# QuantumLiquids/PEPS

Hardware: AMD Instinct MI355X
Metric: configuration-amplitudes/sec (higher is better)
Workload: dtype f32

## Files before the change

### include/pepsgpu.h

```cpp
#ifndef PEPSGPU_H
#define PEPSGPU_H

#include <stddef.h>
#include <stdint.h>

#ifdef __cplusplus
extern "C" {
#endif

typedef struct pepsgpu_ctx pepsgpu_ctx;

enum {
  PEPSGPU_OK = 0,
  PEPSGPU_EINVAL = 1,
  PEPSGPU_EHIP = 2,
  PEPSGPU_ESTATE = 3,
  PEPSGPU_ERANGE = 4,
  PEPSGPU_EEMPTY = 5
};
enum { PEPSGPU_F32 = 0, PEPSGPU_F64 = 1, PEPSGPU_C128 = 3 };
enum { PEPSGPU_LEFT = 0, PEPSGPU_DOWN = 1, PEPSGPU_RIGHT = 2, PEPSGPU_UP = 3 };
enum { PEPSGPU_HORIZONTAL = 0, PEPSGPU_VERTICAL = 1 };
enum { PEPSGPU_SVD_COMPRESS = 0, PEPSGPU_VARIATION2SITE = 1, PEPSGPU_VARIATION1SITE = 2 };

// ... 119 lines not shown
int pepsgpu_sr_weighted_sum(pepsgpu_ctx *ctx, const double *y, double *out);
int pepsgpu_sr_copy_samples(pepsgpu_ctx *ctx, void *dst_samples_dev, int32_t *dst_configs_dev);

int pepsgpu_update_local(pepsgpu_ctx *ctx, int n_sites, const int32_t *sites, const int32_t *new_states,
                         const uint8_t *accept_mask);
int pepsgpu_erase_envs_after_update(pepsgpu_ctx *ctx, int row, int col);

int pepsgpu_evaluate_amplitude(pepsgpu_ctx *ctx, double *out_amp);

int pepsgpu_walker_flags(pepsgpu_ctx *ctx, int32_t *flags_out);
int pepsgpu_sync(pepsgpu_ctx *ctx);
int pepsgpu_stats(pepsgpu_ctx *ctx, double *stats_out, int n);
int pepsgpu_profile_enable(pepsgpu_ctx *ctx, int on);
int pepsgpu_profile_read(pepsgpu_ctx *ctx, double *out);

int pepsgpu_comm_unique_id(void *id128_out);
int pepsgpu_comm_init(pepsgpu_ctx *ctx, int nranks, int rank, const void *id128);
int pepsgpu_comm_size(pepsgpu_ctx *ctx);
int pepsgpu_comm_rank(pepsgpu_ctx *ctx);
int pepsgpu_comm_destroy(pepsgpu_ctx *ctx);
int pepsgpu_allreduce(pepsgpu_ctx *ctx, void *buf, long n, int dtype, int op, int on_device);
int pepsgpu_grad_allreduce(pepsgpu_ctx *ctx);
int pepsgpu_bcast_state(pepsgpu_ctx *ctx, int root);
int pepsgpu_grad_device_ptr(pepsgpu_ctx *ctx, void **so_dev, void **seo_dev, long *n_elems);

int pepsgpu_diag_tgemm(int dtype_in, int dtype_out, const int *desc_ints, int n_ints, const void *A, size_t a_elems,
                       const void *B, size_t b_elems, void *C, size_t c_elems, int nbatch, long wA, long wB, long wC);
int pepsgpu_diag_tgemm_desc(int types, const int *desc_ints, int n_ints, const long *desc_longs, int n_longs,
                            const double *desc_dbls, int n_dbls, const int32_t *pool, long pool_n, const float *scale_in,
                            const void *A, size_t a_elems, long a_offset, const void *B, size_t b_elems, long b_offset,
                            void *C, size_t c_elems, float *scale_out, double *norm_log, int32_t *norm_flag,
                            int32_t *route_out, unsigned long long *flops_out);
int pepsgpu_diag_tgemm_route(int types, const int *desc_ints, int n_ints, const long *desc_longs, int n_longs,
                             const double *desc_dbls, int n_dbls, long a_offset, long b_offset, int32_t *route_out);
int pepsgpu_diag_tgemm_chain3(const int *dims8, const int *site_strides4, long slot, int nslots, const int32_t *sel, int sel_inc,
                              const int32_t *live4, const int32_t *skip, int nbatch, const int *offs3, const float *mps1,
                              const float *bten, const float *site, const float *mps2, float *out, int32_t *flags_out,
                              int32_t *launched_out, int32_t *variant_out);
int pepsgpu_diag_dot4(int dtype, const void *a, const void *b, const int *dims4, int nbatch, const double *lsum, const int32_t *flag,
                      double *out);
int pepsgpu_diag_chol(int dtype_out, const double *G, int n, int nbatch, void *R_out);
int pepsgpu_diag_gram_cols(int dtype, const void *P, int K, int n, int nbatch, const int32_t *klive, double *G_out);
int pepsgpu_diag_gram_rows(const float *M, int n, int K, int nbatch, const int32_t *nrows, double *G_out);
int pepsgpu_diag_mgemm_dense(const float *R, const float *Tt, int m, int la, int a_dim, int u_dim, int k2_dim, int tt_u_inner, int nbatch,
                             const int32_t *m_live, const int32_t *a_live, const int32_t *k2_live, float *M_out);
int pepsgpu_diag_cg_stats(double *out16);
int pepsgpu_diag_lds_gram_chol(int which, const float *X, int n, int K, int nbatch, const int32_t *nlive, float *R_out, int32_t *mlive_out);
int pepsgpu_diag_chol_pivot(const float *X, int n, int K, int nbatch, const int32_t *nlive, int kcap, float *R_out, int32_t *mlive_out);
int pepsgpu_diag_rows_qr(const float *X, int k, int len, int nbatch, const int32_t *klive, float *V_out, int32_t *klive_out);
int pepsgpu_diag_suwa_todo(const double *weights, int n, int init, const uint32_t *words, int steps, int32_t *out_chain);
int pepsgpu_diag_tgemm_chain(const int *dims7, const int32_t *live3_per_entry, int nbatch, const float *R, const float *A,
                             const float *W, float *P_out, int32_t *flags_out);
int pepsgpu_diag_gram_chol(int dtype, const void *P, int K, int n, int nbatch, void *R_out, int32_t *mlive_out);
int pepsgpu_diag_chol_adaptive(int dtype_out, const double *G, int n, int nbatch, void *R_out, int32_t *mlive_out);
int pepsgpu_diag_jacobi(int dtype, void *M, int m, int len, int nbatch, int k, void *Vt_out, void *S_out,
                        int force_global, int *sweeps_out);
const char *pepsgpu_version(void);

#ifdef __cplusplus
}
#endif
#endif
```

### peps_amd/capi.py

```python
import ctypes as C
import os

import numpy as np

_HERE = os.path.dirname(os.path.abspath(__file__))
LIB_PATH = os.environ.get("PEPSGPU_LIB") or os.path.join(_HERE, "lib", "libpepsgpu.so")

F32, F64 = 0, 1
C128 = 3
LEFT, DOWN, RIGHT, UP = 0, 1, 2, 3
HORIZONTAL, VERTICAL = 0, 1
LEFTUP_TO_RIGHTDOWN, LEFTDOWN_TO_RIGHTUP = 0, 1
SVD_COMPRESS, VARIATION2SITE, VARIATION1SITE = 0, 1, 2

_ERR = {1: ValueError, 2: RuntimeError, 3: RuntimeError, 4: IndexError, 5: RuntimeError}

SYMBOLS = [
    "pepsgpu_ctx_create", "pepsgpu_set_truncate_params", "pepsgpu_ctx_destroy", "pepsgpu_last_error", "pepsgpu_state_upload",
    "pepsgpu_walkers_set_configs", "pepsgpu_walkers_get_configs", "pepsgpu_n_walkers",
    "pepsgpu_grow_bmps_step", "pepsgpu_grow_full_bmps", "pepsgpu_grow_bmps_for_row", "pepsgpu_grow_bmps_for_col",
    "pepsgpu_shift_bmps_window", "pepsgpu_delete_inner_bmps", "pepsgpu_bmps_park", "pepsgpu_bmps_unpark", "pepsgpu_generate_bmps_approach",
    "pepsgpu_sweep_slice_exchange", "pepsgpu_sweep_slice_exchange_tab", "pepsgpu_sweep_slice_fullspace", "pepsgpu_sweep_slice_tnn3", "pepsgpu_diag_tnn3_table", "pepsgpu_nn_exchange_slice", "pepsgpu_nn_exchange_slice_tab", "pepsgpu_onsite_slice", "pepsgpu_nnn_exchange_slice", "pepsgpu_diag_nnn_slice_calls", "pepsgpu_nnn_hop_slice_fermion", "pepsgpu_diag_nnn_hop_slice_calls", "pepsgpu_diag_fermion_hop_cand", "pepsgpu_link_exchange_slice", "pepsgpu_diag_link_slice_calls", "pepsgpu_diag_link_cand", "pepsgpu_walker_create", "pepsgpu_walker_clone", "pepsgpu_walker_destroy", "pepsgpu_walker_info", "pepsgpu_walker_set_mpo", "pepsgpu_walker_set_mpo_excited", "pepsgpu_walker_trace_slice", "pepsgpu_diag_walker_slice_calls", "pepsgpu_walker_evolve",
    "pepsgpu_walker_evolve_step", "pepsgpu_walker_contract_row", "pepsgpu_walker_init_bten", "pepsgpu_walker_grow_bten_step",
    "pepsgpu_walker_shift_bten_window", "pepsgpu_walker_trace_with_bten", "pepsgpu_walker_clear_bten", "pepsgpu_walker_get_bmps_tensor",
    "pepsgpu_bmps_stack_size", "pepsgpu_get_bmps_tensor", "pepsgpu_init_bten", "pepsgpu_grow_full_bten",
    "pepsgpu_grow_bten_step", "pepsgpu_shift_bten_window", "pepsgpu_truncate_bten", "pepsgpu_bten_stack_size",
    "pepsgpu_trace", "pepsgpu_replace_nn_trace", "pepsgpu_replace_one_trace", "pepsgpu_punch_hole",
    "pepsgpu_init_bten2", "pepsgpu_grow_full_bten2", "pepsgpu_grow_bten2_step", "pepsgpu_shift_bten2_window",
    "pepsgpu_bten2_stack_size", "pepsgpu_replace_nnn_trace", "pepsgpu_replace_tnn_trace",
    "pepsgpu_bten2_select_set", "pepsgpu_cfg_override_slice", "pepsgpu_replace_plaquette_trace",
    "pepsgpu_replace_sqrt5_trace",
    "pepsgpu_grad_reset", "pepsgpu_grad_accumulate", "pepsgpu_grad_accumulate_states", "pepsgpu_grad_read", "pepsgpu_grad_device_ptr", "pepsgpu_grad_allreduce", "pepsgpu_bcast_state",
    "pepsgpu_comm_unique_id", "pepsgpu_comm_init", "pepsgpu_comm_size", "pepsgpu_comm_rank", "pepsgpu_comm_destroy",
    "pepsgpu_allreduce",
    "pepsgpu_sr_begin", "pepsgpu_sr_append", "pepsgpu_sr_count", "pepsgpu_sr_sum", "pepsgpu_sr_matvec", "pepsgpu_sr_matvec_c128",
    "pepsgpu_sr_cg_solve", "pepsgpu_sr_gram", "pepsgpu_sr_weighted_sum", "pepsgpu_sr_copy_samples",
    "pepsgpu_update_local", "pepsgpu_erase_envs_after_update", "pepsgpu_evaluate_amplitude",
    "pepsgpu_walker_flags", "pepsgpu_sync", "pepsgpu_stats", "pepsgpu_profile_enable", "pepsgpu_profile_read",
    "pepsgpu_diag_tgemm", "pepsgpu_diag_tgemm_desc", "pepsgpu_diag_tgemm_route", "pepsgpu_diag_tgemm_chain", "pepsgpu_diag_tgemm_chain3", "pepsgpu_diag_chol", "pepsgpu_diag_chol_adaptive", "pepsgpu_diag_chol_pivot", "pepsgpu_diag_rows_qr", "pepsgpu_diag_suwa_todo", "pepsgpu_diag_dot4", "pepsgpu_diag_gram_chol", "pepsgpu_diag_gram_cols", "pepsgpu_diag_gram_rows", "pepsgpu_diag_mgemm_dense", "pepsgpu_diag_jacobi", "pepsgpu_version",
]


def load_library(path=LIB_PATH):
    if not os.path.exists(path):
        raise ImportError("libpepsgpu.so not built (%s): run `python -c 'import __graft_entry__ as g; g.build()'`" % path)
    lib = C.CDLL(path)
    vp, ip, dp = C.c_void_p, C.POINTER(C.c_int32), C.POINTER(C.c_double)
    lib.pepsgpu_ctx_create.argtypes = [C.POINTER(vp)] + [C.c_int] * 8 + [C.c_double, C.c_int, C.c_int]
    lib.pepsgpu_set_truncate_params.argtypes = [vp, C.c_int, C.c_int, C.c_double, C.c_int, C.c_double, C.c_int]
    lib.pepsgpu_ctx_destroy.argtypes = [vp]
    lib.pepsgpu_ctx_destroy.restype = None
    lib.pepsgpu_last_error.argtypes = [vp]
    lib.pepsgpu_last_error.restype = C.c_char_p
    lib.pepsgpu_version.restype = C.c_char_p
    lib.pepsgpu_state_upload.argtypes = [vp, vp, C.c_int]
    lib.pepsgpu_walkers_set_configs.argtypes = [vp, C.c_int, ip]
    lib.pepsgpu_walkers_get_configs.argtypes = [vp, ip]
    lib.pepsgpu_n_walkers.argtypes = [vp]
    for name in ("grow_bmps_step", "grow_full_bmps", "grow_bmps_for_row", "grow_bmps_for_col", "shift_bmps_window",
                 "delete_inner_bmps", "generate_bmps_approach", "bmps_stack_size", "bten_stack_size",
                 "grow_bten_step", "shift_bten_window"):
        getattr(lib, "pepsgpu_" + name).argtypes = [vp, C.c_int]
    lib.pepsgpu_bmps_park.argtypes = [vp, C.c_int, C.c_int]
    lib.pepsgpu_bmps_unpark.argtypes = [vp, C.c_int]
    lib.pepsgpu_get_bmps_tensor.argtypes = [vp, C.c_int, C.c_int, C.c_int, ip, dp, dp]
    lib.pepsgpu_init_bten.argtypes = [vp, C.c_int, C.c_int]
    lib.pepsgpu_truncate_bten.argtypes = [vp, C.c_int, C.c_int]
    lib.pepsgpu_grow_full_bten.argtypes = [vp, C.c_int, C.c_int, C.c_int, C.c_int]
    lib.pepsgpu_trace.argtypes = [vp, C.c_int, C.c_int, C.c_int, dp]
    lib.pepsgpu_replace_nn_trace.argtypes = [vp, C.c_int, C.c_int, C.c_int, C.c_int, ip, dp]
    lib.pepsgpu_replace_one_trace.argtypes = [vp, C.c_int, C.c_int, C.c_int, C.c_int, ip, dp]
    lib.pepsgpu_punch_hole.argtypes = [vp, C.c_int, C.c_int, C.c_int, dp]
    for name in ("init_bten2", "grow_bten2_step", "shift_bten2_window"):
        getattr(lib, "pepsgpu_" + name).argtypes = [vp, C.c_int, C.c_int]
    lib.pepsgpu_grow_full_bten2.argtypes = [vp, C.c_int, C.c_int, C.c_int, C.c_int]
    lib.pepsgpu_bten2_stack_size.argtypes = [vp, C.c_int]
    lib.pepsgpu_replace_nnn_trace.argtypes = [vp, C.c_int, C.c_int, C.c_int, C.c_int, C.c_int, ip, dp]
    lib.pepsgpu_bten2_select_set.argtypes = [vp, C.c_int]
    lib.pepsgpu_cfg_override_slice.argtypes = [vp, C.c_int, C.c_int, ip]
    lib.pepsgpu_replace_plaquette_trace.argtypes = [vp, C.c_int, C.c_int, C.c_int, ip, C.c_int, C.c_int, dp]
    lib.pepsgpu_replace_tnn_trace.argtypes = [vp, C.c_int, C.c_int, C.c_int, C.c_int, ip, dp]
    lib.pepsgpu_replace_sqrt5_trace.argtypes = [vp, C.c_int, C.c_int, C.c_int, C.c_int, C.c_int, ip, dp]
    lib.pepsgpu_grad_reset.argtypes = [vp]
    lib.pepsgpu_grad_accumulate.argtypes = [vp, dp, dp, C.c_int]
    lib.pepsgpu_grad_accumulate_states.argtypes = [vp, dp, dp, C.c_int, ip]
    lib.pepsgpu_grad_read.argtypes = [vp, dp, dp]
    lib.pepsgpu_grad_device_ptr.argtypes = [vp, C.POINTER(vp), C.POINTER(vp), C.POINTER(C.c_long)]
    lib.pepsgpu_grad_allreduce.argtypes = [vp]
    lib.pepsgpu_bcast_state.argtypes = [vp, C.c_int]
    lib.pepsgpu_comm_unique_id.argtypes = [vp]
    lib.pepsgpu_comm_init.argtypes = [vp, C.c_int, C.c_int, vp]
    lib.pepsgpu_comm_size.argtypes = [vp]
# ... 658 lines not shown

def diag_tgemm_chain(R, A, W, live):
    R = np.ascontiguousarray(R, dtype=np.float32); A = np.ascontiguousarray(A, dtype=np.float32)
    W = np.ascontiguousarray(W, dtype=np.float32)
    nb, m, l, a = R.shape
    _, _, p, a2 = A.shape
    l2, u = W.shape[3], W.shape[4]
    dims = np.array([m, l, a, p, a2, l2, u], dtype=np.int32)
    lv = np.ascontiguousarray(live, dtype=np.int32)
    P = np.zeros((nb, m, u, l2, a2), dtype=np.float32)
    fl = np.zeros(nb, dtype=np.int32)
    f = lib().pepsgpu_diag_tgemm_chain
    f.argtypes = [C.POINTER(C.c_int32), C.POINTER(C.c_int32), C.c_int, C.c_void_p, C.c_void_p, C.c_void_p, C.c_void_p, C.POINTER(C.c_int32)]
    rc = f(_ip(dims), _ip(lv), nb, R.ctypes.data_as(C.c_void_p), A.ctypes.data_as(C.c_void_p), W.ctypes.data_as(C.c_void_p),
           P.ctypes.data_as(C.c_void_p), _ip(fl))
    if rc != 0:
        raise RuntimeError("diag_tgemm_chain failed: %s" % lib().pepsgpu_last_error(None).decode())
    return P, fl


def diag_chol(dtype_out, G):
    G = np.ascontiguousarray(G, dtype=np.float64)
    nb, n, _ = G.shape
    R = np.zeros((nb, n, n), dtype=np.float32 if dtype_out == F32 else np.float64)
    rc = lib().pepsgpu_diag_chol(dtype_out, _dp(G), n, nb, R.ctypes.data_as(C.c_void_p))
    if rc != 0:
        raise RuntimeError("diag_chol failed: %s" % lib().pepsgpu_last_error(None).decode())
    return R


def diag_chol_adaptive(dtype_out, G):
    G = np.ascontiguousarray(G, dtype=np.float64)
    nb, n, _ = G.shape
    R = np.zeros((nb, n, n), dtype=np.float32 if dtype_out == F32 else np.float64)
    ml = np.zeros(nb, dtype=np.int32)
    rc = lib().pepsgpu_diag_chol_adaptive(dtype_out, _dp(G), n, nb, R.ctypes.data_as(C.c_void_p), _ip(ml))
    if rc != 0:
        raise RuntimeError("diag_chol_adaptive failed: %s" % lib().pepsgpu_last_error(None).decode())
    return R, ml


def diag_gram_chol(dtype, P):
    t = np.float32 if dtype == F32 else np.float64
    P = np.ascontiguousarray(P, dtype=t)
    nb, K, n = P.shape
    R = np.zeros((nb, n, n), dtype=t)
    ml = np.zeros(nb, dtype=np.int32)
    rc = lib().pepsgpu_diag_gram_chol(dtype, P.ctypes.data_as(C.c_void_p), K, n, nb, R.ctypes.data_as(C.c_void_p), _ip(ml))
    if rc != 0:
        raise RuntimeError("diag_gram_chol failed: %s" % lib().pepsgpu_last_error(None).decode())
    return R, ml


def diag_gram_cols(dtype, P, klive=None):
    t = np.float32 if dtype == F32 else np.float64
    P = np.ascontiguousarray(P, dtype=t)
    nb, K, n = P.shape
    G = np.zeros((nb, n, n), dtype=np.float64)
    kl = None if klive is None else np.ascontiguousarray(klive, dtype=np.int32)
    f = lib().pepsgpu_diag_gram_cols
    f.argtypes = [C.c_int, C.c_void_p, C.c_int, C.c_int, C.c_int, C.POINTER(C.c_int32), C.POINTER(C.c_double)]
    rc = f(dtype, P.ctypes.data_as(C.c_void_p), K, n, nb, None if kl is None else _ip(kl), _dp(G))
    if rc != 0:
        raise RuntimeError("diag_gram_cols failed: %s" % lib().pepsgpu_last_error(None).decode())
    return G


def diag_gram_rows(M, nrows):
    M = np.ascontiguousarray(M, dtype=np.float32)
    nb, n, K = M.shape
    G = np.zeros((nb, n, n), dtype=np.float64)
    nr = np.ascontiguousarray(nrows, dtype=np.int32)
    f = lib().pepsgpu_diag_gram_rows
    f.argtypes = [C.c_void_p, C.c_int, C.c_int, C.c_int, C.POINTER(C.c_int32), C.POINTER(C.c_double)]
    rc = f(M.ctypes.data_as(C.c_void_p), n, K, nb, _ip(nr), _dp(G))
    if rc != 0:
        raise RuntimeError("diag_gram_rows failed: %s" % lib().pepsgpu_last_error(None).decode())
    return G


def diag_lds_gram_chol(which, X, nlive):
    X = np.ascontiguousarray(X, dtype=np.float32)
    nb = X.shape[0]
    n, K = (X.shape[1], X.shape[2]) if which == 0 else (X.shape[2], X.shape[1])
    R = np.zeros((nb, n, n), dtype=np.float32)
    ml = np.zeros(nb, dtype=np.int32)
    nl = np.ascontiguousarray(nlive, dtype=np.int32)
    f = lib().pepsgpu_diag_lds_gram_chol
    f.argtypes = [C.c_int, C.c_void_p, C.c_int, C.c_int, C.c_int, C.POINTER(C.c_int32), C.c_void_p, C.POINTER(C.c_int32)]
    rc = f(which, X.ctypes.data_as(C.c_void_p), n, K, nb, _ip(nl), R.ctypes.data_as(C.c_void_p), _ip(ml))
    if rc != 0:
        raise RuntimeError("diag_lds_gram_chol failed: %s" % lib().pepsgpu_last_error(None).decode())
    return R, ml


def diag_chol_pivot(X, nlive, kcap=64):
    X = np.ascontiguousarray(X, dtype=np.float32)
    nb, n, K = X.shape
    R = np.zeros((nb, kcap, n), dtype=np.float32)
    ml = np.zeros(nb, dtype=np.int32)
    nl = np.ascontiguousarray(nlive, dtype=np.int32)
    f = lib().pepsgpu_diag_chol_pivot
    f.argtypes = [C.c_void_p, C.c_int, C.c_int, C.c_int, C.POINTER(C.c_int32), C.c_int, C.c_void_p, C.POINTER(C.c_int32)]
    rc = f(X.ctypes.data_as(C.c_void_p), n, K, nb, _ip(nl), kcap, R.ctypes.data_as(C.c_void_p), _ip(ml))
    if rc != 0:
        raise RuntimeError("diag_chol_pivot failed: %s" % lib().pepsgpu_last_error(None).decode())
# ... 249 lines not shown
```

### peps_amd/csrc/capi.hip

```cpp
#include <cstring>
#include "../../include/pepsgpu.h"
#include "engine_impl.h"
#include "engine_nnn.h"
#include "engine_sr.h"
#include "engine_var.h"
#include "engine_cplx.h"
#include "engine_walker.h"
#include "engine_sweep.h"
#include "comm.h"

using namespace pepsgpu;

namespace pepsgpu {
bool tgemm_use_mfma() {
  static int v = -1;
  if (v < 0) {
    const char *e = getenv("PEPSGPU_NO_MFMA");
    v = (e && e[0] == '1') ? 0 : 1;
  }
  return v == 1;
}
}

struct pepsgpu_ctx {
// ... 681 lines not shown
  const size_t lsm = chol_lowrank_smem_bytes(n), smem = chol_smem_bytes(n);
  allow_dynamic_lds(reinterpret_cast<const void *>(&chol_lowrank_kernel<T>), lsm);
  allow_dynamic_lds(reinterpret_cast<const void *>(&chol_upper_kernel<T>), smem);
  hipLaunchKernelGGL(chol_lowrank_kernel<T>, dim3(nbatch), dim3(256), lsm, 0, (const double *)dG, (long)n * n, n, dR,
                     (long)n * n, dml);
  PG_CHECK_HIP(hipGetLastError());
  launch_chol_upper<T>(0, nbatch, dG, (long)n * n, n, dR, (long)n * n, dml, 1);
  PG_CHECK_HIP(hipGetLastError());
  PG_CHECK_HIP(hipDeviceSynchronize());
  PG_CHECK_HIP(hipMemcpy(Rout, dR, ne * sizeof(T), hipMemcpyDeviceToHost));
  PG_CHECK_HIP(hipMemcpy(mlive, dml, nbatch * sizeof(int), hipMemcpyDeviceToHost));
  (void)hipFree(dG); (void)hipFree(dR); (void)hipFree(dml);
}
extern "C" int pepsgpu_diag_chol_adaptive(int dtype_out, const double *G, int n, int nbatch, void *R_out, int32_t *mlive_out) {
  return guarded(nullptr, [&]() {
    if (dtype_out == 0) diag_chol_adaptive_t<float>(G, n, nbatch, R_out, mlive_out);
    else diag_chol_adaptive_t<double>(G, n, nbatch, R_out, mlive_out);
  });
}
template <typename T, int KCAP>
static void diag_gram_chol_t(const void *P, int K, int n, int nbatch, void *Rout, int32_t *mlive) {
  T *dP, *dR;
  int *dml;
  PG_REQUIRE(n <= 256, 1, "n too large for the fused low-rank kernel");
  PG_CHECK_HIP(hipMalloc(&dP, (size_t)K * n * nbatch * sizeof(T)));
  PG_CHECK_HIP(hipMalloc(&dR, (size_t)n * n * nbatch * sizeof(T)));
  PG_CHECK_HIP(hipMalloc(&dml, nbatch * sizeof(int)));
  PG_CHECK_HIP(hipMemcpy(dP, P, (size_t)K * n * nbatch * sizeof(T), hipMemcpyHostToDevice));
  PG_CHECK_HIP(hipMemset(dR, 0, (size_t)n * n * nbatch * sizeof(T)));
  const int npass = K > KCAP ? 4 : 1;
  std::vector<int> hk(nbatch, 0);
  for (int b = 0; b < nbatch; ++b)
    for (int r = 0; r < K; ++r) {
      const T *row = (const T *)P + ((size_t)b * K + r) * n;
      for (int c = 0; c < n; ++c)
        if (row[c] != T(0)) { hk[b] = r + 1; break; }
    }
  int *dk;
  PG_CHECK_HIP(hipMalloc(&dk, nbatch * sizeof(int)));
  PG_CHECK_HIP(hipMemcpy(dk, hk.data(), nbatch * sizeof(int), hipMemcpyHostToDevice));
  launch_gram_chol_lowrank<T, KCAP>(0, nbatch, (const T *)dP, (long)K * n, n, (const int *)dk, 1, K, dR, (long)n * n, dml, 1,
                                    (const int *)nullptr, npass);
  PG_CHECK_HIP(hipDeviceSynchronize());
  (void)hipFree(dk);
  PG_CHECK_HIP(hipDeviceSynchronize());
  PG_CHECK_HIP(hipMemcpy(Rout, dR, (size_t)n * n * nbatch * sizeof(T), hipMemcpyDeviceToHost));
  PG_CHECK_HIP(hipMemcpy(mlive, dml, nbatch * sizeof(int), hipMemcpyDeviceToHost));
  (void)hipFree(dP); (void)hipFree(dR); (void)hipFree(dml);
}
extern "C" int pepsgpu_diag_gram_chol(int dtype, const void *P, int K, int n, int nbatch, void *R_out, int32_t *mlive_out) {
  return guarded(nullptr, [&]() {
    if (dtype == 0) diag_gram_chol_t<float, 96>(P, K, n, nbatch, R_out, mlive_out);
    else diag_gram_chol_t<double, 48>(P, K, n, nbatch, R_out, mlive_out);
  });
}
template <typename T>
static void diag_gram_cols_t(const void *P, int K, int n, int nbatch, const int32_t *klive, double *G) {
  T *dP;
  double *dG;
  int *dk = nullptr;
  PG_CHECK_HIP(hipMalloc(&dP, (size_t)K * n * nbatch * sizeof(T)));
  PG_CHECK_HIP(hipMalloc(&dG, (size_t)n * n * nbatch * sizeof(double)));
  PG_CHECK_HIP(hipMemcpy(dP, P, (size_t)K * n * nbatch * sizeof(T), hipMemcpyHostToDevice));
  PG_CHECK_HIP(hipMemset(dG, 0, (size_t)n * n * nbatch * sizeof(double)));
  if (klive) {
    PG_CHECK_HIP(hipMalloc(&dk, nbatch * sizeof(int)));
    PG_CHECK_HIP(hipMemcpy(dk, klive, nbatch * sizeof(int), hipMemcpyHostToDevice));
  }
  launch_gram_cols_f64<T>(0, nbatch, (const T *)dP, (long)K * n, n, n, (const int *)dk, 1, K, dG, (const int *)nullptr, 1,
                          (const int *)nullptr, (unsigned long long *)nullptr, (unsigned long long *)nullptr);
  PG_CHECK_HIP(hipDeviceSynchronize());
  PG_CHECK_HIP(hipMemcpy(G, dG, (size_t)n * n * nbatch * sizeof(double), hipMemcpyDeviceToHost));
  (void)hipFree(dP); (void)hipFree(dG); if (dk) (void)hipFree(dk);
}
extern "C" int pepsgpu_diag_gram_cols(int dtype, const void *P, int K, int n, int nbatch, const int32_t *klive, double *G_out) {
  return guarded(nullptr, [&]() {
    PG_REQUIRE(K >= 1 && n >= 1 && n <= 256 && nbatch >= 1, 1, "bad sizes");
    if (dtype == 0) diag_gram_cols_t<float>(P, K, n, nbatch, klive, G_out); else diag_gram_cols_t<double>(P, K, n, nbatch, klive, G_out);
  });
}
extern "C" int pepsgpu_diag_gram_rows(const float *M, int n, int K, int nbatch, const int32_t *nrows, double *G_out) {
  return guarded(nullptr, [&]() {
    PG_REQUIRE(n >= 1 && n <= 256 && K >= 16 && K % 16 == 0 && nbatch >= 1 && nrows, 1, "bad sizes");
    float *dM; double *dG; int *dn;
    const size_t ne = (size_t)n * K * nbatch;
    PG_CHECK_HIP(hipMalloc(&dM, ne * sizeof(float)));
    PG_CHECK_HIP(hipMalloc(&dG, (size_t)n * n * nbatch * sizeof(double)));
    PG_CHECK_HIP(hipMalloc(&dn, nbatch * sizeof(int)));
    PG_CHECK_HIP(hipMemcpy(dM, M, ne * sizeof(float), hipMemcpyHostToDevice));
    PG_CHECK_HIP(hipMemcpy(dn, nrows, nbatch * sizeof(int), hipMemcpyHostToDevice));
    PG_CHECK_HIP(hipMemset(dG, 0, (size_t)n * n * nbatch * sizeof(double)));
    launch_gram_rows_f64<float>(0, nbatch, dM, (long)n * K, K, n, dn, dG, (long)n * n, n, nullptr, nullptr, nullptr);
    PG_CHECK_HIP(hipDeviceSynchronize());
    PG_CHECK_HIP(hipMemcpy(G_out, dG, (size_t)n * n * nbatch * sizeof(double), hipMemcpyDeviceToHost));
    (void)hipFree(dM); (void)hipFree(dG); (void)hipFree(dn);
  });
}
extern "C" int pepsgpu_diag_mgemm_dense(const float *R, const float *Tt, int m, int la, int a_dim, int u_dim, int k2_dim, int tt_u_inner,
                                        int nbatch, const int32_t *m_live, const int32_t *a_live, const int32_t *k2_live, float *M_out) {
  return guarded(nullptr, [&]() {
    const int uk = u_dim * k2_dim;
    float *dR, *dT, *dM;
    int *dl[3] = {nullptr, nullptr, nullptr};
    const int32_t *hl[3] = {m_live, a_live, k2_live};
    PG_CHECK_HIP(hipMalloc(&dR, (size_t)m * la * nbatch * sizeof(float)));
    PG_CHECK_HIP(hipMalloc(&dT, (size_t)la * uk * nbatch * sizeof(float)));
// ... 239 lines not shown
```

### peps_amd/csrc/linalg.h

```cpp
#pragma once
#include "common.h"
#include "cplx.h"

namespace pepsgpu {

template <typename T> struct Eps;
template <> struct Eps<float> { static constexpr float v = 5.9604645e-8f; };
template <> struct Eps<double> { static constexpr double v = 1.1102230246251565e-16; };
template <typename R> struct Eps<cplx<R>> { static constexpr R v = Eps<R>::v; };
__device__ double g_eps64_rt = 1.1102230246251565e-16;
__device__ double g_eps32_rt = 5.9604644775390625e-8;
template <typename T> __device__ __forceinline__ double eps_rt() { return (double)Eps<T>::v; }
template <> __device__ __forceinline__ double eps_rt<float>() { return g_eps32_rt; }
template <> __device__ __forceinline__ double eps_rt<double>() { return g_eps64_rt; }

__device__ __forceinline__ double jr_rcp64(const double x) {
  double r = __builtin_amdgcn_rcp(x);
  r = r * (2.0 - x * r);
  r = r * (2.0 - x * r);
  return r * (2.0 - x * r);
}
__device__ __forceinline__ double jr_rsq64(const double x) {
  double r = __builtin_amdgcn_rsq(x);
  r = r * (1.5 - 0.5 * x * r * r);
// ... 867 lines not shown
        }
#pragma unroll
        for (int jb = 0; jb < RC; jb += 8) {
          if (jb < nl) {
#pragma unroll
            for (int j = jb; j < jb + 8; ++j) {
              if (j < nl) {
                const double rf = gw_readlane_f64(qq[j], lf);
                g0 = fma(-rf, q0[j], g0);
                g1 = fma(-rf, q1[j], g1);
              }
            }
          }
        }
      };
      if (f < 64) step(p0, q0, d0); else step(p1, q1, d1);
      g0 += h0; g1 += h1;
      const double inv = jr_rsq64(piv);
      const double v0 = (ok0 && c0 >= f) ? g0 * inv : 0.0, v1 = (ok1 && c1 >= f) ? g1 * inv : 0.0;
#pragma unroll
      for (int jb = 0; jb < RC; jb += 8) {
        if ((nl & ~7) == jb) {
#pragma unroll
          for (int j = jb; j < jb + 8; ++j) { q0[j] = (j == nl) ? v0 : q0[j]; q1[j] = (j == nl) ? v1 : q1[j]; }
        }
      }
      if (c0 > f) d0 -= v0 * v0;
      if (c1 > f) d1 -= v1 * v1;
      const float a = wave_sum_dpp((float)(v0 * v0 + v1 * v1));
      if (lane == nl) nrm_mine = a;
      ++nl;
    }
    k0 += npr;
    if (k0 >= Ktot) break;
  }
  const float fro = wave_sum_dpp(lane < nl ? nrm_mine : 0.f);
  const bool keep = lane < nl && (double)nrm_mine > eT * eT * (double)fro;
  const unsigned long long km = __ballot(keep);
  const int pos = keep ? __popcll(km & ((1ull << lane) - 1ull)) : -1;
  if (lane == 0) mlive_out[b] = __popcll(km);
  const double sc = maxd > 0.0 ? 1.0 / sqrt(maxd) : 1.0;
#pragma unroll
  for (int j = 0; j < RC; ++j) {
    if (j < nl) {
      const int pj = __builtin_amdgcn_readlane(pos, j);
      if (pj >= 0) {
        if (ok0) Rout[(long)pj * n + r0] = (float)(q0[j] * sc);
        if (ok1) Rout[(long)pj * n + r1] = (float)(q1[j] * sc);
      }
    }
  }
}

template <typename T>
inline void launch_colgram_chol(hipStream_t s, int nbatch, const T *P, long wP, int n, const int *kdyn, int kdyn_mul, int kmax,
                                T *R, long wR, int *mlive, int inner, const int *inner_live, int decline_code, bool hint_dense);

template <typename T, int KCAP>
inline void launch_gram_chol_lowrank(hipStream_t s, int nbatch, const T *P, long wP, int n, const int *kdyn, int kdyn_mul,
                                     int kmax, T *R, long wR, int *mlive, int inner, const int *inner_live,
                                     int max_pass = 1, bool hint_dense = false, int *scratch_list = nullptr) {
  constexpr bool no_narrow = false;
  const bool narrow = !no_narrow && (inner_live != nullptr || n <= 128);
  constexpr int KCAP_S = sizeof(T) == 4 ? 64 : 32;
  constexpr bool short_on = true;
  constexpr bool no_wave_static = false;
  const bool wave_static = sizeof(T) == 4 && !no_wave_static && kdyn == nullptr && kmax <= 64 && true;
  const bool short_first = narrow && short_on && (kdyn != nullptr || wave_static);
  bool first_done = false;
  if constexpr (sizeof(T) == 4) {
    constexpr bool no_cg = false;
    if (!no_cg && hint_dense && inner > 0 && n % inner == 0) {
      launch_colgram_chol<T>(s, nbatch, P, wP, n, kdyn, kdyn_mul, kmax, R, wR, mlive, inner, inner_live, -4, hint_dense);
      first_done = true;
    }
  }
  if (short_first && !first_done) {
    constexpr bool no_wave = false;
    bool done = false;
    if constexpr (sizeof(T) == 4) {
      if (!no_wave) {
        constexpr bool no_list = false;
        int *dl = no_list ? nullptr : scratch_list;
        if (dl) PG_CHECK_HIP(hipMemsetAsync(dl + nbatch, 0, sizeof(int), s));
        hipLaunchKernelGGL(gram_chol_wave_kernel, dim3((nbatch + 3) / 4), dim3(256), 0, s, (const float *)P, wP, n, kdyn, kdyn_mul, kmax,
                           (float *)R, wR, mlive, inner, inner_live, std::max(max_pass, 2), nbatch, dl);
        done = true;
        if (dl && narrow && n <= 128) {
          hipLaunchKernelGGL((gram_chol_lowrank_list_kernel<T, KCAP, 128>), dim3(std::min(nbatch, 512)), dim3(128), 0, s, P, wP, n, kdyn,
                             kdyn_mul, kmax, R, wR, mlive, inner, inner_live, 2, max_pass, (const int *)dl, (const int *)(dl + nbatch));
          PG_CHECK_HIP(hipGetLastError());
          return;
        }
      }
    }
    if (!done)
      hipLaunchKernelGGL((gram_chol_lowrank_kernel<T, KCAP_S, 128, 3, 16>), dim3(nbatch), dim3(128), 0, s, P, wP, n, kdyn, kdyn_mul, kmax,
                         R, wR, mlive, inner, inner_live, 0, std::max(max_pass, 2), 1);
  }
  const bool handed = short_first || first_done;
  if (narrow)
    hipLaunchKernelGGL((gram_chol_lowrank_kernel<T, KCAP, 128>), dim3(nbatch), dim3(128), 0, s, P, wP, n, kdyn, kdyn_mul, kmax,
                       R, wR, mlive, inner, inner_live, handed ? 2 : 0, max_pass, 0);
  if (!narrow || n > 128)
    hipLaunchKernelGGL((gram_chol_lowrank_kernel<T, KCAP, 256>), dim3(nbatch), dim3(256), 0, s, P, wP, n, kdyn, kdyn_mul, kmax,
                       R, wR, mlive, inner, inner_live, narrow ? 1 : (first_done ? 2 : 0), max_pass, 0);
  PG_CHECK_HIP(hipGetLastError());
}

template <typename T>
__global__ __launch_bounds__(256) void adopt_rows_flagged_kernel(const T *__restrict__ Pg, long wP, int cols,
                                                                 const int *__restrict__ kdyn, int kdyn_mul, int kmax,
                                                                 T *__restrict__ Rg, long wR, int *__restrict__ mlive,
                                                                 int inner = 1, const int *__restrict__ inner_live = nullptr) {
  if (mlive[blockIdx.x] >= 0) return;
  const int ilive = inner_live ? inner_live[blockIdx.x] : inner;
  __shared__ double s_red[4];
  const int tid = threadIdx.x, lane = tid & 63, wave = tid >> 6;
  const int K = kdyn ? max(0, min(kmax, kdyn[blockIdx.x] * kdyn_mul)) : kmax;
  const T *P = Pg + (long)blockIdx.x * wP;
  T *R = Rg + (long)blockIdx.x * wR;
  const long cnt = (long)K * cols;
  double a = 0.0;
  for (long e = tid; e < cnt; e += 256) { const double x = (e % inner) < ilive ? (double)P[e] : 0.0; a += x * x; }
  a = wave_sum(a);
  if (lane == 0) s_red[wave] = a;
  __syncthreads();
  const double nrm2 = s_red[0] + s_red[1] + s_red[2] + s_red[3];
  const double sc = nrm2 > 0.0 ? 1.0 / sqrt(nrm2) : 1.0;
  for (long e = tid; e < cnt; e += 256) R[e] = (e % inner) < ilive ? T((double)P[e] * sc) : T(0);
  if (tid == 0) mlive[blockIdx.x] = K;
}

template <typename T>
__global__ __launch_bounds__(256) void zero_dead_cols_kernel(T *__restrict__ Pg, long wP, int cols,
                                                             const int *__restrict__ kdyn, int kdyn_mul, int kmax,
                                                             int inner, const int *__restrict__ inner_live,
                                                             const int *__restrict__ flag) {
// ... 707 lines not shown
```

Before: 125,400.

## Add split-half wave Gram-Cholesky kernel with permlane32 swaps and make it default

Adds a new wave-level pivoted Gram-Cholesky kernel in which the two half-waves each hold alternate K rows of the panel. Partial dot products are combined with permlane32 swaps, and ds_bpermute prefetch overlaps with the FP64 FMAs. It is selected by default through an environment switch in the low-rank launch path, and a diagnostic C API entry is added for testing it. The aim is to halve per-lane register footprint and load/compute latency in the pivot dot loop, at the cost of extra cross-lane swaps and a new code path that must match the old numerics.

```diff
diff --git a/include/pepsgpu.h b/include/pepsgpu.h
--- a/include/pepsgpu.h
+++ b/include/pepsgpu.h
@@ -195,6 +195,8 @@
 int pepsgpu_diag_tgemm_chain(const int *dims7, const int32_t *live3_per_entry, int nbatch, const float *R, const float *A,
                              const float *W, float *P_out, int32_t *flags_out);
 int pepsgpu_diag_gram_chol(int dtype, const void *P, int K, int n, int nbatch, void *R_out, int32_t *mlive_out);
+int pepsgpu_diag_gram_chol_wave(const float *P, int K, int n, int nbatch, const int32_t *klive, int inner,
+                                const int32_t *inner_live, int max_pass, int form, float *R_out, int32_t *mlive_out);
 int pepsgpu_diag_chol_adaptive(int dtype_out, const double *G, int n, int nbatch, void *R_out, int32_t *mlive_out);
 int pepsgpu_diag_jacobi(int dtype, void *M, int m, int len, int nbatch, int k, void *Vt_out, void *S_out,
                         int force_global, int *sweeps_out);
diff --git a/peps_amd/capi.py b/peps_amd/capi.py
--- a/peps_amd/capi.py
+++ b/peps_amd/capi.py
@@ -37,7 +37,7 @@
     "pepsgpu_sr_cg_solve", "pepsgpu_sr_gram", "pepsgpu_sr_weighted_sum", "pepsgpu_sr_copy_samples",
     "pepsgpu_update_local", "pepsgpu_erase_envs_after_update", "pepsgpu_evaluate_amplitude",
     "pepsgpu_walker_flags", "pepsgpu_sync", "pepsgpu_stats", "pepsgpu_profile_enable", "pepsgpu_profile_read",
-    "pepsgpu_diag_tgemm", "pepsgpu_diag_tgemm_desc", "pepsgpu_diag_tgemm_route", "pepsgpu_diag_tgemm_chain", "pepsgpu_diag_tgemm_chain3", "pepsgpu_diag_chol", "pepsgpu_diag_chol_adaptive", "pepsgpu_diag_chol_pivot", "pepsgpu_diag_rows_qr", "pepsgpu_diag_suwa_todo", "pepsgpu_diag_dot4", "pepsgpu_diag_gram_chol", "pepsgpu_diag_gram_cols", "pepsgpu_diag_gram_rows", "pepsgpu_diag_mgemm_dense", "pepsgpu_diag_jacobi", "pepsgpu_version",
+    "pepsgpu_diag_tgemm", "pepsgpu_diag_tgemm_desc", "pepsgpu_diag_tgemm_route", "pepsgpu_diag_tgemm_chain", "pepsgpu_diag_tgemm_chain3", "pepsgpu_diag_chol", "pepsgpu_diag_chol_adaptive", "pepsgpu_diag_chol_pivot", "pepsgpu_diag_rows_qr", "pepsgpu_diag_suwa_todo", "pepsgpu_diag_dot4", "pepsgpu_diag_gram_chol", "pepsgpu_diag_gram_chol_wave", "pepsgpu_diag_gram_cols", "pepsgpu_diag_gram_rows", "pepsgpu_diag_mgemm_dense", "pepsgpu_diag_jacobi", "pepsgpu_version",
 ]
 
 
@@ -802,6 +802,24 @@
     return R, ml
 
 
+def diag_gram_chol_wave(P, klive, inner=1, inner_live=None, max_pass=3, form=1, fill=0.0):
+    P = np.ascontiguousarray(P, dtype=np.float32)
+    nb, K, n = P.shape
+    kl = np.ascontiguousarray(klive, dtype=np.int32)
+    il = None if inner_live is None else np.ascontiguousarray(inner_live, dtype=np.int32)
+    assert kl.shape == (nb,) and (il is None or il.shape == (nb,))
+    R = np.full((nb, n, n), fill, dtype=np.float32)
+    ml = np.zeros(nb, dtype=np.int32)
+    f = lib().pepsgpu_diag_gram_chol_wave
+    fp = C.POINTER(C.c_float)
+    f.argtypes = [fp, C.c_int, C.c_int, C.c_int, C.POINTER(C.c_int32), C.c_int, C.POINTER(C.c_int32), C.c_int, C.c_int, fp,
+                  C.POINTER(C.c_int32)]
+    rc = f(P.ctypes.data_as(fp), K, n, nb, _ip(kl), inner, None if il is None else _ip(il), max_pass, form, R.ctypes.data_as(fp), _ip(ml))
+    if rc != 0:
+        raise RuntimeError("diag_gram_chol_wave failed: %s" % lib().pepsgpu_last_error(None).decode())
+    return R, ml
+
+
 def diag_gram_cols(dtype, P, klive=None):
     t = np.float32 if dtype == F32 else np.float64
     P = np.ascontiguousarray(P, dtype=t)
diff --git a/peps_amd/csrc/capi.hip b/peps_amd/csrc/capi.hip
--- a/peps_amd/csrc/capi.hip
+++ b/peps_amd/csrc/capi.hip
@@ -757,6 +757,47 @@
   return guarded(nullptr, [&]() {
     if (dtype == 0) diag_gram_chol_t<float, 96>(P, K, n, nbatch, R_out, mlive_out);
     else diag_gram_chol_t<double, 48>(P, K, n, nbatch, R_out, mlive_out);
+  });
+}
+extern "C" int pepsgpu_diag_gram_chol_wave(const float *P, int K, int n, int nbatch, const int32_t *klive, int inner,
+                                           const int32_t *inner_live, int max_pass, int form, float *R_out, int32_t *mlive_out) {
+  return guarded(nullptr, [&]() {
+    PG_REQUIRE(K >= 1 && n >= 1 && n <= 256 && nbatch >= 1 && inner >= 1 && n % inner == 0 && max_pass >= 1 && klive, 1, "bad sizes");
+    PG_REQUIRE(form == 0 || form == 1, 1, "form is 0 or 1");
+    const size_t np = (size_t)K * n * nbatch, nr = (size_t)n * n * nbatch;
+    float *dP, *dR;
+    int *dml, *dk, *dil = nullptr, *dl;
+    PG_CHECK_HIP(hipMalloc(&dP, np * sizeof(float)));
+    PG_CHECK_HIP(hipMalloc(&dR, nr * sizeof(float)));
+    PG_CHECK_HIP(hipMalloc(&dml, nbatch * sizeof(int)));
+    PG_CHECK_HIP(hipMalloc(&dk, nbatch * sizeof(int)));
+    PG_CHECK_HIP(hipMalloc(&dl, (nbatch + 1) * sizeof(int)));
+    PG_CHECK_HIP(hipMemcpy(dP, P, np * sizeof(float), hipMemcpyHostToDevice));
+    PG_CHECK_HIP(hipMemcpy(dR, R_out, nr * sizeof(float), hipMemcpyHostToDevice));
+    PG_CHECK_HIP(hipMemcpy(dk, klive, nbatch * sizeof(int), hipMemcpyHostToDevice));
+    PG_CHECK_HIP(hipMemset(dml, 0xff, nbatch * sizeof(int)));
+    PG_CHECK_HIP(hipMemset(dl, 0, (nbatch + 1) * sizeof(int)));
+    if (inner_live) {
+      PG_CHECK_HIP(hipMalloc(&dil, nbatch * sizeof(int)));
+      PG_CHECK_HIP(hipMemcpy(dil, inner_live, nbatch * sizeof(int), hipMemcpyHostToDevice));
+    }
+    const auto wave_kernel = form ? gram_chol_wave_split_kernel : gram_chol_wave_kernel;
+    hipLaunchKernelGGL(wave_kernel, dim3((nbatch + 3) / 4), dim3(256), 0, 0, (const float *)dP, (long)K * n, n, (const int *)dk, 1, K, dR,
+                       (long)n * n, dml, inner, (const int *)dil, max_pass, nbatch, dl);
+    PG_CHECK_HIP(hipGetLastError());
+    if (n <= 128)
+      hipLaunchKernelGGL((gram_chol_lowrank_list_kernel<float, 96, 128>), dim3(std::min(nbatch, 512)), dim3(128), 0, 0, (const float *)dP,
+                         (long)K * n, n, (const int *)dk, 1, K, dR, (long)n * n, dml, inner, (const int *)dil, 2, max_pass, (const int *)dl,
+                         (const int *)(dl + nbatch));
+    else
+      hipLaunchKernelGGL((gram_chol_lowrank_list_kernel<float, 96, 256>), dim3(std::min(nbatch, 512)), dim3(256), 0, 0, (const float *)dP,
+                         (long)K * n, n, (const int *)dk, 1, K, dR, (long)n * n, dml, inner, (const int *)dil, 2, max_pass, (const int *)dl,
+                         (const int *)(dl + nbatch));
+    PG_CHECK_HIP(hipGetLastError());
+    PG_CHECK_HIP(hipDeviceSynchronize());
+    PG_CHECK_HIP(hipMemcpy(R_out, dR, nr * sizeof(float), hipMemcpyDeviceToHost));
+    PG_CHECK_HIP(hipMemcpy(mlive_out, dml, nbatch * sizeof(int), hipMemcpyDeviceToHost));
+    (void)hipFree(dP); (void)hipFree(dR); (void)hipFree(dml); (void)hipFree(dk); (void)hipFree(dl); if (dil) (void)hipFree(dil);
   });
 }
 template <typename T>
diff --git a/peps_amd/csrc/linalg.h b/peps_amd/csrc/linalg.h
--- a/peps_amd/csrc/linalg.h
+++ b/peps_amd/csrc/linalg.h
@@ -943,6 +943,215 @@
   }
 }
 
+__device__ __forceinline__ void gw_swap32(float &a, float &b) {
+  const auto p = __builtin_amdgcn_permlane32_swap(__builtin_bit_cast(unsigned, a), __builtin_bit_cast(unsigned, b), false, false);
+  a = __builtin_bit_cast(float, (unsigned)p[0]);
+  b = __builtin_bit_cast(float, (unsigned)p[1]);
+}
+__device__ __forceinline__ void gw_swap32_f64(double &a, double &b) {
+  const auto pl = __builtin_amdgcn_permlane32_swap((unsigned)__double2loint(a), (unsigned)__double2loint(b), false, false);
+  const auto ph = __builtin_amdgcn_permlane32_swap((unsigned)__double2hiint(a), (unsigned)__double2hiint(b), false, false);
+  a = __hiloint2double((int)ph[0], (int)pl[0]);
+  b = __hiloint2double((int)ph[1], (int)pl[1]);
+}
+template <int S, int PS>
+__device__ __forceinline__ void gw_split_dot(const float (&pp)[4][32], const int K, const int addr, double (&acc)[4]) {
+  constexpr int CH = 4;
+  int pf[2][CH];
+#pragma unroll
+  for (int i = 0; i < CH; ++i) pf[0][i] = __builtin_amdgcn_ds_bpermute(addr, __builtin_bit_cast(int, pp[PS][i]));
+#pragma unroll
+  for (int jb = 0; jb < 32; jb += CH) {
+    if (2 * jb >= K) break;
+    const int cur = (jb / CH) & 1;
+    if (jb + CH < 32) {
+#pragma unroll
+      for (int i = 0; i < CH; ++i) pf[cur ^ 1][i] = __builtin_amdgcn_ds_bpermute(addr, __builtin_bit_cast(int, pp[PS][jb + CH + i]));
+    }
+    __builtin_amdgcn_sched_barrier(0);
+#pragma unroll
+    for (int i = 0; i < CH; ++i) {
+      const double pfd = (double)__builtin_bit_cast(float, pf[cur][i]);
+      double x[S];
+#pragma unroll
+      for (int s = 0; s < S; ++s) asm volatile("v_cvt_f64_f32_e32 %0, %1" : "=v"(x[s]) : "v"(pp[s][jb + i]));
+#pragma unroll
+      for (int s = 0; s < S; ++s) acc[s] = fma(pfd, x[s], acc[s]);
+    }
+  }
+}
+
+__global__ __launch_bounds__(256, 2) void gram_chol_wave_split_kernel(const float *__restrict__ Pg, long wP, int n,
+                                                                    const int *__restrict__ kdyn, int kdyn_mul, int kmax,
+                                                                    float *__restrict__ Rg, long wR, int *__restrict__ mlive_out,
+                                                                    int inner, const int *__restrict__ inner_live, int max_pass,
+                                                                    int nbatch, int *__restrict__ decl_list = nullptr) {
+  constexpr int KC = 64, RC = 16, KH = KC / 2;
+  const int lane = threadIdx.x & 63;
+  const int b = __builtin_amdgcn_readfirstlane(blockIdx.x * 4 + (threadIdx.x >> 6));
+  if (b >= nbatch) return;
+  const int Ktot = kdyn ? max(0, min(kmax, kdyn[b] * kdyn_mul)) : kmax;
+  const int ilive = inner_live ? min(inner, inner_live[b]) : inner;
+  const int ncols = (n / inner) * ilive;
+  if (Ktot > KC + (max_pass - 1) * (KC - RC) || ncols > 128) {
+    if (lane == 0) { mlive_out[b] = -4; if (decl_list) decl_list[atomicAdd(decl_list + nbatch, 1)] = b; }
+    return;
+  }
+  const int nslot = (ncols + 31) >> 5;
+  const float *P = Pg + (long)b * wP;
+  float *Rout = Rg + (long)b * wR;
+  const int c0 = lane, c1 = lane + 64;
+  const bool ok0 = c0 < ncols, ok1 = c1 < ncols;
+  const int r0 = ok0 ? (c0 / ilive) * inner + (c0 % ilive) : 0, r1 = ok1 ? (c1 / ilive) * inner + (c1 % ilive) : 0;
+  const int hp = lane >> 5, lh = lane & 31;
+  unsigned rs[4];
+#pragma unroll
+  for (int s = 0; s < 4; ++s) {
+    const int c = lh + 32 * s;
+    rs[s] = c < ncols ? (unsigned)((c / ilive) * inner + (c % ilive)) : 0u;
+  }
+  const double eT = NOISE_C * (double)Eps<float>::v;
+  float pp[4][KH];
+  double q0[RC], q1[RC];
+#pragma unroll
+  for (int j = 0; j < RC; ++j) { q0[j] = 0.0; q1[j] = 0.0; }
+  int nl = 0, k0 = 0;
+  double maxd = 0.0;
+  float nrm_mine = 0.f;
+#pragma unroll 1
+  for (int pass = 0;; ++pass) {
+    const int nfr = nl;
+    const int npr = min(Ktot - k0, KC - (pass > 0 ? RC : 0));
+    const int K = __builtin_amdgcn_readfirstlane(nfr + npr);
+    double d0 = 0.0, d1 = 0.0;
+    const int klast = max(K - 1, nfr);
+#pragma unroll
+    for (int j = 0; j < KH; ++j) {
+      const unsigned ro = (unsigned)((k0 + min(max(2 * j + hp, nfr), klast) - nfr) * n);
+#pragma unroll
+      for (int s = 0; s < 4; ++s) pp[s][j] = P[ro + rs[s]];
+    }
+#pragma unroll
+    for (int j = 0; j < KH; ++j) {
+      gw_swap32(pp[0][j], pp[1][j]);
+      gw_swap32(pp[2][j], pp[3][j]);
+#pragma unroll
+      for (int h = 0; h < 2; ++h) {
+        const int k = 2 * j + h;
+        float x0 = (k < K && ok0) ? pp[h][j] : 0.f, x1 = (k < K && ok1) ? pp[2 + h][j] : 0.f;
+        if (k < RC && k < nfr) { x0 = (float)q0[k < RC ? k : 0]; x1 = (float)q1[k < RC ? k : 0]; }
+        pp[h][j] = x0; pp[2 + h][j] = x1;
+        d0 = fma((double)x0, (double)x0, d0);
+        d1 = fma((double)x1, (double)x1, d1);
+      }
+      gw_swap32(pp[0][j], pp[1][j]);
+      gw_swap32(pp[2][j], pp[3][j]);
+    }
+#pragma unroll
+    for (int j = 0; j < RC; ++j) { q0[j] = 0.0; q1[j] = 0.0; }
+    {
+      double md = fmax(d0, d1);
+#pragma unroll
+      for (int o = 32; o > 0; o >>= 1) md = fmax(md, __shfl_xor(md, o, 64));
+      maxd = md;
+    }
+    const double thresh = fmax((double)n * 2.220446049250313e-16, eT * eT) * maxd;
+    int f = -1;
+    nl = 0;
+    nrm_mine = 0.f;
+#pragma unroll 1
+    for (;;) {
+      int cand = (ok0 && c0 > f && d0 > thresh) ? c0 : ((ok1 && c1 > f && d1 > thresh) ? c1 : 0x7fffffff);
+      cand = wave_min_dpp(cand);
+      if (cand == 0x7fffffff || nl >= K) break;
+      if (nl == RC) {
+        if (lane == 0) { mlive_out[b] = -4; if (decl_list) decl_list[atomicAdd(decl_list + nbatch, 1)] = b; }
+        return;
+      }
+      f = __builtin_amdgcn_readfirstlane(cand);
+      const int lf = f & 63;
+      double acc[4] = {0.0, 0.0, 0.0, 0.0};
+      {
+        const int addr = ((lane & 32) | (f & 31)) << 2;
+        const int ps = f >> 5;
+        if (nslot == 3) {
+          if (ps == 0) gw_split_dot<3, 0>(pp, K, addr, acc);
+          else if (ps == 1) gw_split_dot<3, 1>(pp, K, addr, acc);
+          else gw_split_dot<3, 2>(pp, K, addr, acc);
+        } else if (nslot == 2) {
+          if (ps == 0) gw_split_dot<2, 0>(pp, K, addr, acc);
+          else gw_split_dot<2, 1>(pp, K, addr, acc);
+        } else if (nslot == 4) {
+          if (ps == 0) gw_split_dot<4, 0>(pp, K, addr, acc);
+          else if (ps == 1) gw_split_dot<4, 1>(pp, K, addr, acc);
+          else if (ps == 2) gw_split_dot<4, 2>(pp, K, addr, acc);
+          else gw_split_dot<4, 3>(pp, K, addr, acc);
+        } else {
+          gw_split_dot<1, 0>(pp, K, addr, acc);
+        }
+      }
+      gw_swap32_f64(acc[0], acc[1]);
+      gw_swap32_f64(acc[2], acc[3]);
+      double g0 = acc[0], h0 = acc[1], g1 = acc[2], h1 = acc[3], piv;
+      auto qsub = [&](const double (&qq)[RC], const double dd) {
+        piv = gw_readlane_f64(dd, lf);
+#pragma unroll
+        for (int jb = 0; jb < RC; jb += 8) {
+          if (jb < nl) {
+#pragma unroll
+            for (int j = jb; j < jb + 8; ++j) {
+              if (j < nl) {
+                const double rf = gw_readlane_f64(qq[j], lf);
+                g0 = fma(-rf, q0[j], g0);
+                g1 = fma(-rf, q1[j], g1);
+              }
+            }
+          }
+        }
+      };
+      if (f < 64) qsub(q0, d0); else qsub(q1, d1);
+      g0 += h0; g1 += h1;
+      const double inv = jr_rsq64(piv);
+      const double v0 = (ok0 && c0 >= f) ? g0 * inv : 0.0, v1 = (ok1 && c1 >= f) ? g1 * inv : 0.0;
+#pragma unroll
+      for (int jb = 0; jb < RC; jb += 8) {
+        if ((nl & ~7) == jb) {
+#pragma unroll
+          for (int j = jb; j < jb + 8; ++j) { q0[j] = (j == nl) ? v0 : q0[j]; q1[j] = (j == nl) ? v1 : q1[j]; }
+        }
+      }
+      if (c0 > f) d0 -= v0 * v0;
+      if (c1 > f) d1 -= v1 * v1;
+      const float a = wave_sum_dpp((float)(v0 * v0 + v1 * v1));
+      if (lane == nl) nrm_mine = a;
+      ++nl;
+    }
+    k0 += npr;
+    if (k0 >= Ktot) break;
+  }
+  const float fro = wave_sum_dpp(lane < nl ? nrm_mine : 0.f);
+  const bool keep = lane < nl && (double)nrm_mine > eT * eT * (double)fro;
+  const unsigned long long km = __ballot(keep);
+  const int pos = keep ? __popcll(km & ((1ull << lane) - 1ull)) : -1;
+  if (lane == 0) mlive_out[b] = __popcll(km);
+  const double sc = maxd > 0.0 ? 1.0 / sqrt(maxd) : 1.0;
+#pragma unroll
+  for (int j = 0; j < RC; ++j) {
+    if (j < nl) {
+      const int pj = __builtin_amdgcn_readlane(pos, j);
+      if (pj >= 0) {
+        if (ok0) Rout[(long)pj * n + r0] = (float)(q0[j] * sc);
+        if (ok1) Rout[(long)pj * n + r1] = (float)(q1[j] * sc);
+      }
+    }
+  }
+}
+
+inline bool factor_split() {
+  static const bool v = getenv("PEPSGPU_FACTOR_SPLIT") ? atoi(getenv("PEPSGPU_FACTOR_SPLIT")) != 0 : true;
+  return v;
+}
+
 template <typename T>
 inline void launch_colgram_chol(hipStream_t s, int nbatch, const T *P, long wP, int n, const int *kdyn, int kdyn_mul, int kmax,
                                 T *R, long wR, int *mlive, int inner, const int *inner_live, int decline_code, bool hint_dense);
@@ -974,7 +1183,8 @@
         constexpr bool no_list = false;
         int *dl = no_list ? nullptr : scratch_list;
         if (dl) PG_CHECK_HIP(hipMemsetAsync(dl + nbatch, 0, sizeof(int), s));
-        hipLaunchKernelGGL(gram_chol_wave_kernel, dim3((nbatch + 3) / 4), dim3(256), 0, s, (const float *)P, wP, n, kdyn, kdyn_mul, kmax,
+        const auto wave_kernel = factor_split() ? gram_chol_wave_split_kernel : gram_chol_wave_kernel;
+        hipLaunchKernelGGL(wave_kernel, dim3((nbatch + 3) / 4), dim3(256), 0, s, (const float *)P, wP, n, kdyn, kdyn_mul, kmax,
                            (float *)R, wR, mlive, inner, inner_live, std::max(max_pass, 2), nbatch, dl);
         done = true;
         if (dl && narrow && n <= 128) {
```

Result: faster. 128,200, median of 6 (+2.2%).
